# hahnyuan/PTQ4ViT

Hardware: AMD Instinct MI355X
Metric: calibration throughput (wrapped modules calibrated per second), ViT-B/224 W8A8, 32 calibration images (higher is better)
Workload: dtype int8

## Files before the change

ptq4vit_amd/csrc/p4v_api.hip:

```cpp
#include <hip/hip_runtime.h>

#include <algorithm>
#include <atomic>
#include <climits>
#include <cstdarg>
#include <cstdio>
#include <condition_variable>
#include <cstring>
#include <deque>
#include <functional>
#include <thread>
#include <mutex>
#include <string>
#include <unordered_map>
#include <type_traits>
#include <vector>

#include "../../include/ptq4vit_hip.h"
#include "../../include/ptq4vit_hip_debug.h"
#include "p4v_kernels.h"

using namespace p4v;

namespace {
// ... 75 lines not shown

struct StatRec { hipEvent_t a, b; int kind; double macs, alg; int stage, gx, gz; double ms, bytes; };
thread_local double g_alg_bytes = 0;
thread_local double g_alg_macs_cand = 0;
thread_local double g_exec_frac = 1.0;
thread_local bool g_stat_on = false;
thread_local std::vector<StatRec> g_stat_recs;
thread_local std::vector<StatRec> g_stat_done;
thread_local bool g_b1_keep = false;
thread_local std::vector<float> g_b1_totals;
enum PruneStage { STAGE_FULL = 0, STAGE_A = 1, STAGE_B1 = 2, STAGE_B2 = 3, STAGE_A2 = 4 };
thread_local int g_stage = STAGE_FULL;
thread_local p4v_kernel_stats g_stats = {};
thread_local long g_memo_hits = 0, g_memo_misses = 0;
std::atomic<long long> g_prune_cnt[4];
constexpr int VARIANT_KEPT = 1 | 2 | 4 | 2048 | 32768 | 65536 | 131072 | 524288 | 1048576 | 2097152 | 4194304 | 8388608 | 134217728;
std::atomic<int> g_variant_word{0};
#define g_variant (g_variant_word.load(std::memory_order_relaxed) & 0x3fffffff)
#define g_force_v1 ((g_variant_word.load(std::memory_order_relaxed) >> 30) & 1)
std::atomic<int> g_tune[16];
enum { TUNE_CG6 = 0, TUNE_CG2 = 1, TUNE_CG2G = 2, TUNE_CG7 = 3, TUNE_PRINT = 4, TUNE_ORDER7 = 5, TUNE_P6 = 6, TUNE_PLANE_GIB = 7, TUNE_EPI6W = 8,
       TUNE_LOOSE_PCT = 9, TUNE_SLICE_DIV = 10, TUNE_SLICE_SMALL = 11, TUNE_B1_PATH = 12, TUNE_TIER2 = 13, TUNE_TIER2_DIV = 14, TUNE_LOOSE_ROWS = 15 };
inline bool tune_b1_removed(int v) { return v == 1 || v == 2 || v == 3 || v == 5 || v == 6 || v == 8 || v == 10 || v == 12; }
inline int tune(int k) { return g_tune[k].load(std::memory_order_relaxed); }
inline bool b1_previous() { return tune(TUNE_B1_PATH) == 4; }

inline int ws_aligned(const void* p) {
    return ((uintptr_t)p % WS_ALIGN) == 0 ? 0 : fail(P4V_ERR_INVALID, "d_workspace must be aligned to %zu bytes", WS_ALIGN);
}

struct Group;
// ... 421 lines not shown
    if (total >= (1L << 31)) return fail(P4V_ERR_UNSUPPORTED, "operand plane too large for k_pack (%ld 16-element runs)", total);
    const int groups = cdiv((p.crange && live_max > 0) ? std::min(p.C, live_max) : p.C, PACK_CG);
    const long cap = !p.crange ? 256L * 64 : live_max > 0 ? std::max(256L * 12, 256L * 64 / groups) : 256L * 12;
    const int blocks = (int)std::min<long>(cdiv(total, 256), cap);
    if (p.mode == PACK_TWIN_I8) {
        if (sizeof(T) != 1 || p.C != 1 || p.c_inner != 0 || !p.scales || p.conv || p.zdiv > 0)
            return fail(P4V_ERR_UNSUPPORTED, "merged twin plane: one fixed row-major int8 plane only");
        return enqueue(c, KERN(PackParams, k_pack_twin), dim3(blocks), dim3(256), 0, p);
    }
    const bool single = sizeof(T) == 1 && pack1_ok(p, live_max) && !g_pack_general.load(std::memory_order_relaxed);
    if (tune(TUNE_PRINT) > 1) fprintf(stderr, "[p4v] %s stage %d: Z %d Rp %d Kp %d C %d crange %d done %d live_max %d layout %d grid %d x %d\n", single ? "k_pack1" : "k_pack", g_stage, p.Z, p.Rp, p.Kp, p.C, p.crange != nullptr, p.done != nullptr, live_max, p.c_inner, blocks, single ? 1 : groups);
    if (single) return enqueue(c, KERN(PackParams, k_pack1), dim3(blocks), dim3(256), 0, p);
    return enqueue(c, KERN_T(PackParams, k_pack, T), dim3(blocks, groups), dim3(256), 0, p);
}

inline int lockstep(const Ctx& c, int kind) {
    if (!c.grp) return 1;
    const int seen = (kind >= 0 && kind < 16) ? c.grp->last_par[kind] : 0;
    return std::max(1, seen > 0 ? seen : c.par);
}
inline int cu_slots(const Ctx& c, int slots, int kind) { return std::max(8, slots / lockstep(c, kind)); }
#define P4V_EPI4(epi, X)                                   \
    switch (epi) {                                         \
        case EPI_SQ_W: { constexpr int E = EPI_SQ_W; X; }  \
        case EPI_SQ: { constexpr int E = EPI_SQ; X; }      \
        case EPI_ABS: { constexpr int E = EPI_ABS; X; }    \
        default: { constexpr int E = EPI_W_SQ; X; }        \
    }

template <typename T, bool TWIN> int launch_sweep_epi(Ctx& c, const SweepParams& p, int epi, int cgroups, const StatInfo* si) {
// ... 47 lines not shown
    HIPCHK(hipStreamSynchronize(c.st));
    std::vector<unsigned long long> h(n);
    HIPCHK(hipMemcpy(h.data(), g_trace, n * 8, hipMemcpyDeviceToHost));
    FILE* f = fopen(getenv("P4V_TRACE_FILE"), "ab");
    unsigned long long hdr[4] = {0xABCDull, grid.x, grid.z, (unsigned long long)ktiles};
    fwrite(hdr, 8, 4, f); fwrite(h.data(), 8, n, f); fclose(f);
    return 0;
}
#endif

inline StatInfo stat_info(int kind, double macs, double alg, int gx, int gz, double bytes) {
    return StatInfo{kind, macs * g_exec_frac, alg * g_exec_frac, g_stage, gx, gz, bytes};
}

enum SweepKind { SK_BOUND, SK_SWEEP6, SK_SWEEP5, SK_SWEEP7, SK_SWEEP7_TWIN, SK_SWEEP7_MERGED, SK_SWEEP9, SK_SWEEP8, SK_SWEEP2G, SK_SWEEP2,
                 SK_GENERIC_I8, SK_GENERIC_F32, SK_COUNT };
constexpr int SWEEP_RECORD_KIND[SK_COUNT] = {12, 2, 5, 3, 4, 4, 6, 7, 8, 9, 0, 1};
inline bool sweep_stationary(SweepKind k) { return k == SK_SWEEP6 || k == SK_SWEEP5; }
inline bool sweep_large_k(SweepKind k) { return k == SK_SWEEP7 || k == SK_SWEEP7_TWIN || k == SK_SWEEP7_MERGED; }

int launch_sweep5(Ctx& c, const Sweep3Params& p, int epi, int cgroups) {
    if (c.dry) return 0;
    const int per = 2 * cdiv(p.c1 - p.c0, 2 * cgroups);
    const size_t lds = (size_t)p.ktiles * SW2_TILE + (size_t)SW5_NP * 2 * SW2_TILE + (size_t)per * 8 * sizeof(float) * 2 + 256;
    dim3 grid(p.stiles * p.ttiles, 1, cgroups), block(512);
#ifdef P4V_TRACE
    CHK(trace_attach(const_cast<Sweep3Params&>(p)));
#endif
    const StatInfo si = stat_info(SWEEP_RECORD_KIND[SK_SWEEP5], (double)p.stiles * 128 * (double)p.ttiles * 128 * (double)p.ldk * (p.c1 - p.c0), g_alg_macs_cand * (p.c1 - p.c0),
                                  (int)grid.x, (int)grid.z, g_alg_bytes);
    const StatInfo* sp = &si;
    P4V_EPI4(epi, CHK(enqueue(c, KERN_T(Sweep3Params, k_sweep5, E), grid, block, lds, p, sp)); break)
// ... 97 lines not shown
    const int per_max = (int)((160 * 1024 - SW7_NS * SW7_STAGE - 256) / 192);
    cgroups = std::max(cgroups, cdiv(nc, per_max));
    const int per = cdiv(nc, cgroups);
    const size_t lds = (size_t)SW7_NS * SW7_STAGE + (size_t)per * 192 + 256;
    Sweep7Params q = p;
    q.cgroups = cgroups;
    dim3 grid(p.rtiles * p.ctiles * cgroups, 1, 1);
    const StatInfo si = stat_info(SWEEP_RECORD_KIND[twin ? SK_SWEEP7_TWIN : SK_SWEEP7], (double)p.rtiles * 256 * (double)p.ctiles * 256 * (double)p.ldk * nc, g_alg_macs_cand * nc,
                                  (int)grid.x, (int)grid.z, g_alg_bytes);
    const StatInfo* sp = &si;
    return twin == 2 ? launch_sweep7_epi<2>(c, q, epi, grid, lds, sp) : twin ? launch_sweep7_epi<1>(c, q, epi, grid, lds, sp) : launch_sweep7_epi<0>(c, q, epi, grid, lds, sp);
}

int launch_sweep(Ctx& c, const SweepParams& p, SweepKind kind, bool twin, int epi, int cgroups) {
    if (c.dry) return 0;
    const double kelems = (double)p.ldk / (kind == SK_GENERIC_F32 ? 4 : 1);
    const int tiles = p.mtiles * p.ntiles;
    auto record = [&](int gx) {
        return stat_info(SWEEP_RECORD_KIND[kind], (double)p.mtiles * SW_BM * (double)p.ntiles * SW_BN * kelems * p.Z * (p.c1 - p.c0) * (twin ? 2 : 1),
                         g_alg_macs_cand * (p.c1 - p.c0), gx, cgroups, g_alg_bytes);
    };
    switch (kind) {
        case SK_BOUND: {
            const bool prev = b1_previous();
            const StatInfo si = record(tiles * (prev ? 2 : 1));
            const dim3 grid(tiles * (prev ? 2 : 1)), block(256);
            if (prev) P4V_EPI4(epi, return enqueue(c, KERN_T(SweepParams, k_bound, E, 1), grid, block, 0, p, &si))
            P4V_EPI4(epi, return enqueue(c, KERN_T(SweepParams, k_bound, E, 2), grid, block, 0, p, &si))
        }
        case SK_SWEEP9: {
            const StatInfo si = record(p.halves);
// ... 6 lines not shown
        case SK_SWEEP2G: {
            const StatInfo si = record(tiles);
            return twin ? launch_sweep2g_epi<true>(c, p, epi, cgroups, &si) : launch_sweep2g_epi<false>(c, p, epi, cgroups, &si);
        }
        case SK_SWEEP2: {
            const StatInfo si = record(tiles);
            return twin ? launch_sweep2_epi<true>(c, p, epi, cgroups, &si) : launch_sweep2_epi<false>(c, p, epi, cgroups, &si);
        }
        case SK_GENERIC_I8: {
            const StatInfo si = record(tiles);
            return twin ? launch_sweep_epi<int8_t, true>(c, p, epi, cgroups, &si) : launch_sweep_epi<int8_t, false>(c, p, epi, cgroups, &si);
        }
        case SK_GENERIC_F32: {
            const StatInfo si = record(tiles);
            return twin ? launch_sweep_epi<float, true>(c, p, epi, cgroups, &si) : launch_sweep_epi<float, false>(c, p, epi, cgroups, &si);
        }
        default: return fail(P4V_ERR_INVALID, "launch_sweep: family %d has a launcher of its own", (int)kind);
    }
}

int launch_finish(Ctx& c, const FinishParams& p) {
    return enqueue(c, KERN(FinishParams, k_finish), dim3(p.C, p.nj), dim3(256), 0, p);
}

int launch_finish_cos(Ctx& c, const FinishCosParams& p) {
    const int gy = p.j_mode == 3 ? cdiv(p.S, 256) : p.nj;
    return enqueue(c, KERN(FinishCosParams, k_finish_cos), dim3(p.C, gy), dim3(p.j_mode == 3 ? 256 : 1024), 0, p);
}

int launch_select(Ctx& c, const SelectParams& p_) {
// ... 224 lines not shown
    CHK(launch_pass_select(c, ps, scores));
    c.ws.off = mark;
    return 0;
}

struct SweepPlan {
    SweepKind kind;
    bool pairs;
    bool merged7;
    bool b64;
    bool fast_cos;
    bool epi6_on;
    const int* rblk;
    const int* rblk_z;
    int esz, Kp, Mp, Np, NpB;
    long row_plane1, col_plane1, exp_plane;
    int chunk, chunk_al; size_t slack;
    int cin_exp, cin_fix;
    size_t zero_bias_n, epi7_n;
    int s6_stiles, s6_ttiles; size_t epi6_bytes;
    bool a_search;
    long part_cs;
    long p_zs, p_cs; int NpP;
    int s3_groups, cos6_Sp;
    int h9;
    long fin_zs; int fin_ld, fin_rows, fin_cols, fin_jdiv;
};

int sweep9_halves(const Pass& ps, int ktiles) {
    const int epi = ps.epi;
    if (ktiles != 1 || ps.twin || ps.row.expanded == ps.col.expanded || epi == EPI_STORE || epi == EPI_FWD || epi == EPI_COS) return 0;
// ... 5 lines not shown
    if (halves > 32 / SW9_NW) return 0;
    const double waste = (double)rup(ps.Mrows, 128) * rup(ps.Ncols, 128) / ((double)rup(ps.Mrows, 16) * rup(ps.Ncols, 16));
    return (waste >= 1.4 || (g_variant & 1048576)) ? halves : 0;
}
bool sweep8_ok(const Pass& ps, int ktiles) {
    return ktiles == 1 && !ps.twin && ps.row.expanded != ps.col.expanded && ps.epi != EPI_STORE && ps.epi != EPI_FWD && ps.epi != EPI_COS &&
           !(g_variant & 65536);
}
bool sweep2g_ok(const Pass& ps, int ktiles) {
    return ps.col.expanded && !ps.row.expanded && ktiles >= 16 && ps.o_bs == 0 && ps.o_nbs == 0 && ps.epi != EPI_COS;
}

int plan_sweep(const Ctx& c, const Pass& ps, SweepPlan& pl) {
    pl = SweepPlan{};
    const int esz = pl.esz = ps.i8 ? 1 : 4;
    const int Kp = pl.Kp = (int)rup(ps.K, 64 / esz);
    const int ktiles = Kp * esz / SW_BKB;
    const long K64 = rup(ps.K, 64);
    const bool cosm = ps.epi == EPI_COS, i8v2 = ps.i8 && !g_force_v1;
    const bool one_expanded = ps.row.expanded != ps.col.expanded, plain_out = ps.o_bs == 0 && ps.o_nbs == 0;
    const bool scale32 = ps.sb_mode != 1 || ps.s_cs == 1 || ps.sb_div % 32 == 0;
    const bool score32 = ps.j_mode == 0 || (ps.j_mode == 1 && (ps.nj == 1 || ps.j_div % 32 == 0));
    const bool blocks64 = (ps.s_cs == 1 || ps.sb_div % 64 == 0) && (ps.j_mode == 0 || (ps.j_mode == 1 && (ps.nj == 1 || ps.j_div % 64 == 0)));
    const bool bound = ps.bound_kernel && i8v2 && !ps.twin && ps.Z == 1 && !ps.stores() && !cosm && plain_out && ps.bias_axis == 0 &&
                       (ps.sb_mode == 0 || ps.sb_mode == 1) && score32 && scale32 && (ps.eq_n == 1 || ps.crange);
    const bool stat_ok = !bound && !ps.stores() && i8v2 && !ps.twin && (!cosm || ps.cos6) && !(g_variant & 4) && ps.Z == 1 &&
                         ps.sb_mode == 1 && blocks64 && one_expanded && K64 <= 768 && plain_out;
    const bool regs6 = stat_ok && sweep6_supported(ktiles);
    if (ps.cos6 && !regs6) return fail(P4V_ERR_UNSUPPORTED, "cosine pass planned for k_sweep6 does not qualify for it");
    const bool big7 = !bound && !stat_ok && !ps.stores() && i8v2 && (!cosm || ps.cos7) && !(g_variant & 32768) && ps.Z == 1 &&
                      K64 >= 1024 && K64 % 256 == 0 && (long)ps.Mrows * ps.o_ms * 4 < (1L << 32) && ps.sb_mode == 1 && scale32 && score32 &&
                      one_expanded && !(ps.twin && (ps.row.expanded || ps.row2.expanded)) &&
                      plain_out && ps.o_ns == 1 && ps.Ncols % 32 == 0 && ps.o_ms % 4 == 0 &&
                      (c.dry || ((((unsigned long long)ps.O) | ((unsigned long long)(ps.G ? ps.G : ps.O))) & 15) == 0) && ps.bias_axis == 0;
    if (ps.cos7 && (!big7 || ps.twin)) return fail(P4V_ERR_UNSUPPORTED, "cosine pass planned for k_sweep7 does not qualify for it");
    const bool fast = !stat_ok && i8v2 && !cosm && scale32 && (score32 || ps.j_mode == 2);
    pl.fast_cos = cosm && !stat_ok && !big7 && i8v2 && !ps.stores() && tune(TUNE_B1_PATH) != 7 && scale32;
    pl.pairs = stat_ok && !regs6;
    pl.merged7 = big7 && ps.twin && ps.twin_disjoint && !(g_variant & 2097152);
    pl.kind = bound ? SK_BOUND : regs6 ? SK_SWEEP6 : stat_ok ? SK_SWEEP5 :
              big7 ? (pl.merged7 ? SK_SWEEP7_MERGED : ps.twin ? SK_SWEEP7_TWIN : SK_SWEEP7) :
              !(fast || pl.fast_cos) ? (ps.i8 ? SK_GENERIC_I8 : SK_GENERIC_F32) :
              (fast && sweep8_ok(ps, ktiles)) ? SK_SWEEP8 : (fast && sweep2g_ok(ps, ktiles)) ? SK_SWEEP2G : SK_SWEEP2;
    const bool blk_ranges = ps.crange && ps.crange_blk && tune(TUNE_B1_PATH) != 9;
    pl.rblk = (blk_ranges && regs6 && !ps.row.expanded && ps.j_mode == 1 && ps.nj == ps.s_cs && ps.j_div == ps.sb_div) ? ps.crange_blk : nullptr;
    pl.rblk_z = (blk_ranges && !stat_ok && ps.j_mode == 2 && ps.nj == ps.j_div && ps.Z > 1 && !cosm && !ps.stores() && !bound && K64 < 1024)
                    ? ps.crange_blk : nullptr;
    const int Mp = pl.Mp = (int)rup(ps.Mrows, big7 ? (ps.twin ? 128 : 256) : (regs6 && !ps.row.expanded) ? 256 : SW_BM);
    const int Np = pl.Np = (int)rup(ps.Ncols, big7 ? 256 : (regs6 && !ps.col.expanded) ? 256 : SW_BM);
    pl.b64 = fast && !big7 && !bound && ps.Z > 1 && !ps.col_zs_shared && ps.Ncols <= 64 && ktiles >= 2 && ktiles <= 15 && !ps.stores();
    pl.NpB = pl.b64 ? 64 : Np;
    pl.row_plane1 = (long)(ps.row_zs_shared ? 1 : ps.Z) * Mp * Kp * esz;
    pl.col_plane1 = (long)(ps.col_zs_shared ? 1 : ps.Z) * pl.NpB * Kp * esz;
    pl.exp_plane = ps.row.expanded ? pl.row_plane1 : pl.col_plane1;
    pl.chunk = (int)std::max<long>(1, std::min<long>(ps.eq_n, PLANE_BUDGET / std::max<long>(1, pl.exp_plane)));
    if (pl.pairs && pl.chunk > 1) pl.chunk &= ~1;
    pl.chunk_al = pl.pairs ? ((pl.chunk + 1) & ~1) : pl.chunk;
    pl.slack = stat_ok ? 4096 : 0;
    pl.cin_exp = bound ? 3 : stat_ok ? (pl.pairs ? 2 : 1) : 0;
    pl.cin_fix = (bound || regs6) ? 3 : 0;
    pl.zero_bias_n = stat_ok ? (size_t)std::max(Mp, Np) : 0;
    pl.epi7_n = big7 ? (size_t)Mp * Np * 2 : 0;
    const bool a_search = pl.a_search = ps.row.expanded;
    pl.s6_stiles = (a_search ? Np : Mp) / 256; pl.s6_ttiles = (int)cdiv(a_search ? ps.Mrows : ps.Ncols, 64);
    pl.epi6_on = regs6 && (a_search || ps.cos6 || tune(TUNE_EPI6W) == 1);
    pl.epi6_bytes = pl.epi6_on ? (size_t)pl.s6_stiles * pl.s6_ttiles * (256 * 64 * 8) : 0;
    const int MT = Mp / 64, s3_slabs = (a_search ? Np : Mp) / 64, s3_groups = pl.s3_groups = (a_search ? Mp : Np) / 32;
    const int NpP = pl.NpP = stat_ok ? s3_groups : fast ? Np / 32 : Np;
    const int MT7 = big7 ? (Mp / (ps.twin ? 128 : 256)) * 4 : 0;
    const bool cosp = ps.cos6 || ps.cos7;
// ... 18 lines not shown
        if (cosp) pl.fin_zs = (long)FS * cos6_Sp * 3;
        pl.fin_ld = cosp ? cos6_Sp : Np; pl.fin_rows = cosp ? FS : MT; pl.fin_cols = cosp ? ps.Mrows : ps.Ncols;
        pl.fin_jdiv = std::max(1, ps.cos_j_div);
    }
    return 0;
}
inline SweepKind chunk_kind(const SweepPlan& pl, int nc) { return (pl.kind == SK_SWEEP2G && nc < 2) ? SK_SWEEP2 : pl.kind; }

struct PassBufs {
    char* row; char* row2; char* col;
    float* part; float* S1; float* S2; float* scores; float* zero_bias; float* epi7; float* epi6;
    PlaneCache* pc; EpiCache* ec;
};
int pass_workspace(Ctx& c, const Pass& ps, const SweepPlan& pl, PassBufs& b) {
    PlaneCache* pc = b.pc = (ps.cache && pl.chunk >= ps.eq_n && !ps.stores() && ps.row.expanded != ps.col.expanded &&
                             !(ps.twin && ps.row2.expanded) && pl.exp_plane * (long)ps.eq_n <= PLANE_CACHE_MAX) ? ps.cache : nullptr;
    if (pc && !pc->assigned) {
        pc->buf = c.ws.get_top((size_t)pl.exp_plane * pl.chunk_al + pl.slack);
        pc->done = reinterpret_cast<unsigned char*>(c.ws.get_top((size_t)rup(ps.eq_n, 256)));
        pc->assigned = true; pc->valid = false;
        if (!c.dry && pc->done) CHK(q_fill(c, pc->done, 0, (size_t)ps.eq_n));
    }
    b.row = ps.row.prepacked ? (char*)ps.row.plane :
            (pc && ps.row.expanded) ? pc->buf : c.ws.get<char>((size_t)pl.row_plane1 * (ps.row.expanded ? pl.chunk_al : 1) + pl.slack);
    b.row2 = !ps.twin ? nullptr : ps.row2.prepacked ? (char*)ps.row2.plane : c.ws.get<char>((size_t)pl.row_plane1 * (ps.row2.expanded ? pl.chunk : 1));
    b.col = ps.col.prepacked ? (char*)ps.col.plane :
            (pc && ps.col.expanded) ? pc->buf : c.ws.get<char>((size_t)pl.col_plane1 * (ps.col.expanded ? pl.chunk_al : 1) + pl.slack);
    b.part = c.ws.get<float>((size_t)pl.part_cs * ps.eq_n);
    b.S1 = !ps.use_s1 ? nullptr : ps.S1_pre ? ps.S1_pre : c.ws.get<float>((size_t)ps.eq_n * ps.s_cs);
    b.S2 = !(ps.use_s1 && ps.twin) ? nullptr : ps.S2_pre ? ps.S2_pre : c.ws.get<float>((size_t)ps.eq_n * ps.s_cs);
    b.scores = ps.scores_keep ? ps.scores_keep : c.ws.get<float>((size_t)ps.eq_n * std::max(1, ps.nj));
    b.zero_bias = (pl.zero_bias_n && !ps.bias) ? c.ws.get<float>(pl.zero_bias_n) : nullptr;
    b.epi7 = pl.epi7_n ? c.ws.get<float>(pl.epi7_n) : nullptr;
    EpiCache* ec = b.ec = (pl.epi6_on && ps.ecache && (long)pl.epi6_bytes <= PLANE_CACHE_MAX) ? ps.ecache : nullptr;
    if (ec && !ec->assigned) {
        ec->buf = c.ws.get_top(pl.epi6_bytes);
        ec->assigned = true; ec->valid = false;
    }
    b.epi6 = !pl.epi6_on ? nullptr : ec ? reinterpret_cast<float*>(ec->buf) : c.ws.get<float>(pl.epi6_bytes / 4);
    if (!c.ws.ok()) return fail(P4V_ERR_WORKSPACE, "workspace too small: need >= %zu bytes", c.ws.off);
    return 0;
}

int pack_operand(Ctx& c, const Pass& ps, const SweepPlan& pl, const PassBufs& b, const Operand& op, char* buf, bool col, int c0, int nc) {
    PackParams pk = op.pk;
    pk.Rp = col ? pl.NpB : pl.Mp; pk.Kp = pl.Kp; pk.dst = buf;
    pk.Z = (col ? ps.col_zs_shared : ps.row_zs_shared) ? 1 : ps.Z;
    pk.C = op.expanded ? nc : 1;
    pk.c_inner = op.expanded ? pl.cin_exp : pl.cin_fix;
    if (op.expanded && pk.scales) pk.scales += (long)c0 * pk.sc_cs;
    if (op.expanded && ps.crange) {
        pk.crange = ps.crange; pk.c_base = c0;
        pk.done = (b.pc && b.pc->done) ? b.pc->done : nullptr;
    }
    int live_max = -1;
    if (pk.crange && ps.host_hi > ps.host_lo) live_max = std::max(0, std::min(ps.host_hi, c0 + nc) - std::max(ps.host_lo, c0));
    else if (pk.crange && ps.host_len > 0) live_max = std::min(ps.host_len, nc);
    return ps.i8 ? launch_pack<int8_t>(c, pk, live_max) : launch_pack<float>(c, pk, live_max);
}
int pack_expanded(Ctx& c, const Pass& ps, const SweepPlan& pl, const PassBufs& b, int c0, int nc) {
    PlaneCache* pc = b.pc;
    const bool packed = pc && pc->valid;
    if (ps.row.expanded && !packed) CHK(pack_operand(c, ps, pl, b, ps.row, b.row, false, c0, nc));
    if (ps.twin && ps.row2.expanded) CHK(pack_operand(c, ps, pl, b, ps.row2, b.row2, false, c0, nc));
    if (ps.col.expanded && !packed) CHK(pack_operand(c, ps, pl, b, ps.col, b.col, true, c0, nc));
    if (pc && !ps.crange && !packed) {
        pc->valid = true;
        if (!c.dry && pc->done) CHK(q_fill(c, pc->done, 1, (size_t)ps.eq_n));
    }
    return 0;
}

// ... 143 lines not shown
    q.ldk = pl.Kp; q.ktiles = pl.Kp / SW_BKB;
    q.S1 = b.S1; q.S2 = b.S2; q.s_cs = ps.s_cs; q.sb_div = ps.s_cs > 1 ? std::max(1, ps.sb_div) : (1 << 30);
    q.E = b.epi7;
    q.c0 = c0; q.c1 = c0 + nc; q.crange = ps.crange;
    q.part = b.part; q.p_cs = pl.p_cs; q.NG = ps.cos7 ? pl.cos6_Sp : pl.NpP;
    q.rtiles = pl.Np / 256; q.ctiles = pl.Mp / (ps.twin ? 128 : 256);
    int cg7 = choose_cgroups((long)q.rtiles * q.ctiles, nc, q.ktiles + 3, cu_slots(c, 256, SWEEP_RECORD_KIND[ps.twin ? SK_SWEEP7_TWIN : SK_SWEEP7]), 6.0, 0.62, 100);
    if (tune(TUNE_CG7) > 0) cg7 = std::max(1, std::min(nc, tune(TUNE_CG7)));
    q.order = tune(TUNE_ORDER7) > 0 ? tune(TUNE_ORDER7) - 1 : 1;
    if (tune(TUNE_PRINT) > 0) fprintf(stderr, "[p4v] sweep7 tiles %d x %d ktiles %d cand %d twin %d -> cgroups %d\n", q.rtiles, q.ctiles, q.ktiles, nc, (int)ps.twin, cg7);
    if (pl.kind == SK_SWEEP7_MERGED) { q.twin_s = ps.row.pk.scales; q.C2 = b.row2; }
    return launch_sweep7(c, q, pl.kind == SK_SWEEP7_MERGED ? 2 : ps.twin ? 1 : 0, ps.epi, cg7);
}

int sweep_chunk_tiled(Ctx& c, const Pass& ps, const SweepPlan& pl, const PassBufs& b, SweepKind kind, int c0, int nc) {
    const int esz = pl.esz, Mp = pl.Mp, Np = pl.Np, Kp = pl.Kp;
    SweepParams sp{};
    sp.a_cs = ps.row.expanded ? pl.row_plane1 : 0;
    sp.A = b.row - (long)c0 * sp.a_cs;
    sp.a_zs = ps.row_zs_shared ? 0 : (long)Mp * Kp * esz;
    if (ps.twin) {
        sp.a2_cs = ps.row2.expanded ? pl.row_plane1 : 0;
        sp.A2 = b.row2 - (long)c0 * sp.a2_cs;
        sp.a2_zs = sp.a_zs;
    }
    sp.b_cs = ps.col.expanded ? pl.col_plane1 : 0;
    sp.B = b.col - (long)c0 * sp.b_cs;
    sp.b_zs = ps.col_zs_shared ? 0 : (long)pl.NpB * Kp * esz;
    sp.b_rows = pl.b64 ? 64 : 0;
    sp.ldk = Kp * esz; sp.ktiles = sp.ldk / SW_BKB;
    sp.S1 = b.S1; sp.S2 = b.S2; sp.s_cs = ps.s_cs; sp.sb_mode = ps.sb_mode; sp.sb_div = std::max(1, ps.sb_div);
    sp.bias = ps.bias; sp.bias_axis = ps.bias_axis; sp.bias_zs = ps.bias_zs;
    sp.O = ps.O; sp.Wt = ps.G ? ps.G : ps.O; sp.wt_mode = ps.wt_mode;
    sp.o_zs = ps.o_zs; sp.o_bs = ps.o_bs; sp.o_ms = ps.o_ms; sp.o_nbs = ps.o_nbs; sp.o_ns = ps.o_ns;
    sp.o_inner = ps.o_inner > 0 ? ps.o_inner : INT_MAX;
    sp.o_ninner = ps.o_ninner > 0 ? ps.o_ninner : INT_MAX;
    sp.M = ps.Mrows; sp.N = ps.Ncols; sp.Z = ps.Z; sp.c0 = c0; sp.c1 = c0 + nc; sp.crange = ps.crange;
    sp.crange_blk = pl.rblk_z; sp.cb_div = std::max(1, ps.j_div);
    sp.part = b.part; sp.p_cs = pl.p_cs; sp.p_zs = pl.p_zs; sp.Np = pl.NpP;
    sp.mtiles = Mp / SW_BM; sp.ntiles = Np / SW_BN;
    sp.dbg = g_variant & 3;
    sp.store = ps.store_out;
    const long wgs = (long)sp.mtiles * sp.ntiles * ps.Z;
    int cgroups;
    switch (kind) {
        case SK_GENERIC_I8: case SK_GENERIC_F32:
            cgroups = choose_cgroups(wgs, nc, sp.ktiles, cu_slots(c, 512, SWEEP_RECORD_KIND[kind]), 20.0, ps.i8 ? 1.6 : 2.6);
            break;
        case SK_SWEEP9:
            sp.halves = pl.h9;
            sp.rows_p_stream = sp.a_cs == 0 ? Np : Mp;
            cgroups = choose_cgroups((long)pl.h9 * ps.Z, nc, 1, cu_slots(c, SW9_NW == 4 ? 512 : 256, SWEEP_RECORD_KIND[SK_SWEEP9]), 12.0, 0.9);
            break;
        case SK_BOUND:
            sp.bound = 1;
            sp.dbg = tune(TUNE_B1_PATH) >= 16 ? (tune(TUNE_B1_PATH) >> 4) : 0;
            sp.A = b.row; sp.B = b.col; sp.a_cs = sp.b_cs = 0;
            [[fallthrough]];
        default:
            cgroups = choose_cgroups(wgs, nc, sp.ktiles, cu_slots(c, ps.twin ? 256 : 512, SWEEP_RECORD_KIND[SK_SWEEP2]), ps.twin ? 40.0 : 25.0, ps.twin ? 0.45 : 0.40);
    }
    const bool tuned = kind != SK_GENERIC_I8 && kind != SK_GENERIC_F32 && !pl.fast_cos && !ps.stores();
    if (tuned) {
        const char* g = kind == SK_SWEEP2G ? "g" : "";
        if (const int t_ = tune(kind == SK_SWEEP2G ? TUNE_CG2G : TUNE_CG2); t_ > 0) cgroups = std::max(1, std::min(nc, t_));
        if (tune(TUNE_PRINT) > 0) fprintf(stderr, "[p4v] sweep2%s tiles %d x %d z %d ktiles %d cand %d twin %d -> cgroups %d\n", g, sp.mtiles, sp.ntiles, ps.Z, sp.ktiles, nc, (int)ps.twin, cgroups);
    }
    return launch_sweep(c, sp, kind, ps.twin, ps.epi, cgroups);
}

int finish_pass(Ctx& c, const Pass& ps, const SweepPlan& pl, const PassBufs& b) {
    if (ps.epi == EPI_COS) {
        FinishCosParams fp{b.part, pl.p_cs, pl.fin_zs, pl.fin_ld, pl.fin_rows, ps.cos_ZB, ps.cos_ZV, pl.fin_cols, ps.eq_n,
                           ps.cos_j_mode, pl.fin_jdiv, ps.nj, ps.norm, b.scores};
        return launch_finish_cos(c, fp);
    }
    FinishParams fp{b.part, pl.p_cs, pl.fin_zs, pl.fin_ld, pl.fin_rows, ps.Z, pl.fin_cols, ps.eq_n, ps.j_mode, pl.fin_jdiv, ps.nj, ps.norm,
// ... 2756 lines not shown
```

ptq4vit_amd/csrc/p4v_kernels.h:

```cpp
#pragma once
#include <hip/hip_runtime.h>
#include <stdint.h>
#include <type_traits>

namespace p4v {

typedef int v4i __attribute__((ext_vector_type(4)));
typedef int v16i __attribute__((ext_vector_type(16)));
typedef float v4f __attribute__((ext_vector_type(4)));
typedef float v16f __attribute__((ext_vector_type(16)));
typedef float v2f __attribute__((ext_vector_type(2)));

#ifndef P4V_GROUP_KERNARG
#define P4V_GROUP_KERNARG (4096 - 256)
#endif
template <typename P> struct GroupArgs {
    static constexpr int CAP_RAW = (P4V_GROUP_KERNARG - 16) / (int)(sizeof(P) + 16);
    static constexpr int CAP = CAP_RAW > 64 ? 64 : CAP_RAW;
    int n;
    unsigned off[CAP + 1];
    unsigned gx[CAP], gy[CAP], gz[CAP];
    P p[CAP];
};
#define P4V_BIDX uint3{blockIdx.x, blockIdx.y, blockIdx.z}
// ... 933 lines not shown
                nn += __shfl_xor(nn, 32);
                oo += __shfl_xor(oo, 32);
                if (g == 0) {
                    float* q = cos_part(p, c, z, mt * 2 + wr, n0 + wc * 32 + l31);
                    q[0] = dot; q[1] = nn; q[2] = oo;
                }
            }
            zero_acc();
        }
    }
}
template <typename T, bool TWIN, int EPI>
__global__ __launch_bounds__(512, 2) void k_sweep(SweepParams p) { k_sweep_body<T, TWIN, EPI>(p, P4V_BIDX, P4V_GDIM); }
template <typename T, bool TWIN, int EPI>
__global__ __launch_bounds__(512, 2) void k_sweep_g(GroupArgs<SweepParams> a) { P4V_GROUP_ENTER(a); k_sweep_body<T, TWIN, EPI>(a.p[m_], vb_, vg_); }

static constexpr int SW2_NS = 4;
static constexpr int SW2_TILE = 128 * 64;

__device__ __forceinline__ void glds16(const void* g, void* l) {
    __builtin_amdgcn_global_load_lds((const __attribute__((address_space(1))) void*)g,
                                     (__attribute__((address_space(3))) void*)l, 16, 0, 0);
}
template <int OFF> __device__ __forceinline__ void glds16_imm(const void* g, void* l) {
    __builtin_amdgcn_global_load_lds((const __attribute__((address_space(1))) void*)g,
                                     (__attribute__((address_space(3))) void*)l, 16, OFF, 0);
}

__device__ __forceinline__ float wave_sum_dpp(float v) {
    auto dpp = [](float x, auto ctrl, auto rmask) __attribute__((always_inline)) {
// ... 3604 lines not shown
```

Before: 689.9.

## Add bf16x3-split MFMA sweep path for fp32 passes with quantized expanded operand

Adds a new sweep kind for non-int8 passes whose expanded column operand is symmetrically quantized to at most 256 levels. That operand is packed as exact bf16 integers, and the raw fp32 row operand is split into three bf16 parts. A new kernel runs bf16 MFMA for the hi and lo parts and applies the candidate scale in the epilogue, replacing the generic fp32 sweep. The aim is to move fp32 GEMM work onto bf16 matrix cores, at the cost of three MFMAs per tile and larger row-plane storage. Precision depends on the three-way split. Workspace sizing is adjusted to fit the new plane sizes.

```diff
diff --git a/ptq4vit_amd/csrc/p4v_api.hip b/ptq4vit_amd/csrc/p4v_api.hip
--- a/ptq4vit_amd/csrc/p4v_api.hip
+++ b/ptq4vit_amd/csrc/p4v_api.hip
@@ -113,7 +113,7 @@
 thread_local p4v_kernel_stats g_stats = {};
 thread_local long g_memo_hits = 0, g_memo_misses = 0;
 std::atomic<long long> g_prune_cnt[4];
-constexpr int VARIANT_KEPT = 1 | 2 | 4 | 2048 | 32768 | 65536 | 131072 | 524288 | 1048576 | 2097152 | 4194304 | 8388608 | 134217728;
+constexpr int VARIANT_KEPT = 1 | 2 | 4 | 16 | 2048 | 32768 | 65536 | 131072 | 524288 | 1048576 | 2097152 | 4194304 | 8388608 | 134217728;
 std::atomic<int> g_variant_word{0};
 #define g_variant (g_variant_word.load(std::memory_order_relaxed) & 0x3fffffff)
 #define g_force_v1 ((g_variant_word.load(std::memory_order_relaxed) >> 30) & 1)
@@ -565,6 +565,17 @@
     return enqueue(c, KERN_T(PackParams, k_pack, T), dim3(blocks, groups), dim3(256), 0, p);
 }
 
+int launch_pack_bf3(Ctx& c, const PackParams& p, bool expanded, int live_max) {
+    if (c.dry) return 0;
+    if (p.crange && live_max == 0) return 0;
+    const long total = (long)p.Z * p.Rp * (p.Kp / 16);
+    if (total >= (1L << 31)) return fail(P4V_ERR_UNSUPPORTED, "operand plane too large for k_pack_bf3 (%ld 16-element runs)", total);
+    if (!expanded) return enqueue(c, KERN(PackParams, k_pack_bf3x), dim3((unsigned)std::min<long>(cdiv(total, 256), 256L * 64)), dim3(256), 0, p);
+    const int groups = cdiv((p.crange && live_max > 0) ? std::min(p.C, live_max) : p.C, PACK_CG);
+    const long cap = !p.crange ? 256L * 64 : live_max > 0 ? std::max(256L * 12, 256L * 64 / groups) : 256L * 12;
+    return enqueue(c, KERN(PackParams, k_pack_bf3q), dim3((unsigned)std::min<long>(cdiv(total, 256), cap), groups), dim3(256), 0, p);
+}
+
 inline int lockstep(const Ctx& c, int kind) {
     if (!c.grp) return 1;
     const int seen = (kind >= 0 && kind < 16) ? c.grp->last_par[kind] : 0;
@@ -642,8 +653,8 @@
 }
 
 enum SweepKind { SK_BOUND, SK_SWEEP6, SK_SWEEP5, SK_SWEEP7, SK_SWEEP7_TWIN, SK_SWEEP7_MERGED, SK_SWEEP9, SK_SWEEP8, SK_SWEEP2G, SK_SWEEP2,
-                 SK_GENERIC_I8, SK_GENERIC_F32, SK_COUNT };
-constexpr int SWEEP_RECORD_KIND[SK_COUNT] = {12, 2, 5, 3, 4, 4, 6, 7, 8, 9, 0, 1};
+                 SK_GENERIC_I8, SK_GENERIC_F32, SK_BF3, SK_COUNT };
+constexpr int SWEEP_RECORD_KIND[SK_COUNT] = {12, 2, 5, 3, 4, 4, 6, 7, 8, 9, 0, 1, 1};
 inline bool sweep_stationary(SweepKind k) { return k == SK_SWEEP6 || k == SK_SWEEP5; }
 inline bool sweep_large_k(SweepKind k) { return k == SK_SWEEP7 || k == SK_SWEEP7_TWIN || k == SK_SWEEP7_MERGED; }
 
@@ -771,7 +782,7 @@
 
 int launch_sweep(Ctx& c, const SweepParams& p, SweepKind kind, bool twin, int epi, int cgroups) {
     if (c.dry) return 0;
-    const double kelems = (double)p.ldk / (kind == SK_GENERIC_F32 ? 4 : 1);
+    const double kelems = kind == SK_BF3 ? 3.0 * p.ldk / 2 : (double)p.ldk / (kind == SK_GENERIC_F32 ? 4 : 1);
     const int tiles = p.mtiles * p.ntiles;
     auto record = [&](int gx) {
         return stat_info(SWEEP_RECORD_KIND[kind], (double)p.mtiles * SW_BM * (double)p.ntiles * SW_BN * kelems * p.Z * (p.c1 - p.c0) * (twin ? 2 : 1),
@@ -808,6 +819,11 @@
         case SK_GENERIC_F32: {
             const StatInfo si = record(tiles);
             return twin ? launch_sweep_epi<float, true>(c, p, epi, cgroups, &si) : launch_sweep_epi<float, false>(c, p, epi, cgroups, &si);
+        }
+        case SK_BF3: {
+            const StatInfo si = record(tiles);
+            const dim3 grid(tiles, p.Z, cgroups), block(512);
+            P4V_EPI4(epi, return enqueue(c, KERN_T(SweepParams, k_sweep_bf3, E), grid, block, 2 * BF3_STAGE, p, &si))
         }
         default: return fail(P4V_ERR_INVALID, "launch_sweep: family %d has a launcher of its own", (int)kind);
     }
@@ -1062,7 +1078,9 @@
     const int* rblk;
     const int* rblk_z;
     int esz, Kp, Mp, Np, NpB;
+    int esz_row, esz_col;
     long row_plane1, col_plane1, exp_plane;
+    long row_alloc1, col_alloc1, exp_alloc;
     int chunk, chunk_al; size_t slack;
     int cin_exp, cin_fix;
     size_t zero_bias_n, epi7_n;
@@ -1098,8 +1116,16 @@
 int plan_sweep(const Ctx& c, const Pass& ps, SweepPlan& pl) {
     pl = SweepPlan{};
     const int esz = pl.esz = ps.i8 ? 1 : 4;
-    const int Kp = pl.Kp = (int)rup(ps.K, 64 / esz);
-    const int ktiles = Kp * esz / SW_BKB;
+    const PackParams& cpk = ps.col.pk;
+    const bool bf3_ok = !ps.i8 && !ps.twin && !ps.stores() && ps.epi != EPI_COS && !ps.use_s1 &&
+                     !ps.row.expanded && !ps.row.prepacked && ps.row.pk.mode == PACK_RAW &&
+                     ps.col.expanded && cpk.mode == PACK_SYM && cpk.hi - cpk.lo <= 255 && cpk.lo >= -128 && cpk.hi <= 128 &&
+                     (cpk.blk_mode == 0 || (cpk.blk_mode == 1 && !cpk.blk_div2 && cpk.blk_div >= 1 && cpk.sc_cs == cpk.nblk_r)) &&
+                     ps.sb_mode == 0 && ps.s_cs == 1;
+    const bool bf3 = bf3_ok && !(g_variant & 16);
+    pl.esz_row = bf3 ? 6 : esz; pl.esz_col = bf3 ? 2 : esz;
+    const int Kp = pl.Kp = (int)rup(ps.K, bf3 ? BF3_BK : 64 / esz);
+    const int ktiles = bf3 ? Kp / BF3_BK : Kp * esz / SW_BKB;
     const long K64 = rup(ps.K, 64);
     const bool cosm = ps.epi == EPI_COS, i8v2 = ps.i8 && !g_force_v1;
     const bool one_expanded = ps.row.expanded != ps.col.expanded, plain_out = ps.o_bs == 0 && ps.o_nbs == 0;
@@ -1124,7 +1150,7 @@
     pl.merged7 = big7 && ps.twin && ps.twin_disjoint && !(g_variant & 2097152);
     pl.kind = bound ? SK_BOUND : regs6 ? SK_SWEEP6 : stat_ok ? SK_SWEEP5 :
               big7 ? (pl.merged7 ? SK_SWEEP7_MERGED : ps.twin ? SK_SWEEP7_TWIN : SK_SWEEP7) :
-              !(fast || pl.fast_cos) ? (ps.i8 ? SK_GENERIC_I8 : SK_GENERIC_F32) :
+              !(fast || pl.fast_cos) ? (ps.i8 ? SK_GENERIC_I8 : bf3 ? SK_BF3 : SK_GENERIC_F32) :
               (fast && sweep8_ok(ps, ktiles)) ? SK_SWEEP8 : (fast && sweep2g_ok(ps, ktiles)) ? SK_SWEEP2G : SK_SWEEP2;
     const bool blk_ranges = ps.crange && ps.crange_blk && tune(TUNE_B1_PATH) != 9;
     pl.rblk = (blk_ranges && regs6 && !ps.row.expanded && ps.j_mode == 1 && ps.nj == ps.s_cs && ps.j_div == ps.sb_div) ? ps.crange_blk : nullptr;
@@ -1134,10 +1160,17 @@
     const int Np = pl.Np = (int)rup(ps.Ncols, big7 ? 256 : (regs6 && !ps.col.expanded) ? 256 : SW_BM);
     pl.b64 = fast && !big7 && !bound && ps.Z > 1 && !ps.col_zs_shared && ps.Ncols <= 64 && ktiles >= 2 && ktiles <= 15 && !ps.stores();
     pl.NpB = pl.b64 ? 64 : Np;
-    pl.row_plane1 = (long)(ps.row_zs_shared ? 1 : ps.Z) * Mp * Kp * esz;
-    pl.col_plane1 = (long)(ps.col_zs_shared ? 1 : ps.Z) * pl.NpB * Kp * esz;
+    pl.row_plane1 = (long)(ps.row_zs_shared ? 1 : ps.Z) * Mp * Kp * pl.esz_row;
+    pl.col_plane1 = (long)(ps.col_zs_shared ? 1 : ps.Z) * pl.NpB * Kp * pl.esz_col;
     pl.exp_plane = ps.row.expanded ? pl.row_plane1 : pl.col_plane1;
-    pl.chunk = (int)std::max<long>(1, std::min<long>(ps.eq_n, PLANE_BUDGET / std::max<long>(1, pl.exp_plane)));
+    pl.row_alloc1 = pl.row_plane1; pl.col_alloc1 = pl.col_plane1;
+    if (bf3_ok) {
+        const long Kf = rup(ps.K, 16), Kb = rup(ps.K, BF3_BK);
+        pl.row_alloc1 = (long)(ps.row_zs_shared ? 1 : ps.Z) * Mp * std::max(Kf * 4, Kb * 6);
+        pl.col_alloc1 = (long)(ps.col_zs_shared ? 1 : ps.Z) * pl.NpB * std::max(Kf * 4, Kb * 2);
+    }
+    pl.exp_alloc = ps.row.expanded ? pl.row_alloc1 : pl.col_alloc1;
+    pl.chunk = (int)std::max<long>(1, std::min<long>(ps.eq_n, PLANE_BUDGET / std::max<long>(1, pl.exp_alloc)));
     if (pl.pairs && pl.chunk > 1) pl.chunk &= ~1;
     pl.chunk_al = pl.pairs ? ((pl.chunk + 1) & ~1) : pl.chunk;
     pl.slack = stat_ok ? 4096 : 0;
@@ -1186,18 +1219,18 @@
 };
 int pass_workspace(Ctx& c, const Pass& ps, const SweepPlan& pl, PassBufs& b) {
     PlaneCache* pc = b.pc = (ps.cache && pl.chunk >= ps.eq_n && !ps.stores() && ps.row.expanded != ps.col.expanded &&
-                             !(ps.twin && ps.row2.expanded) && pl.exp_plane * (long)ps.eq_n <= PLANE_CACHE_MAX) ? ps.cache : nullptr;
+                             !(ps.twin && ps.row2.expanded) && pl.exp_alloc * (long)ps.eq_n <= PLANE_CACHE_MAX) ? ps.cache : nullptr;
     if (pc && !pc->assigned) {
-        pc->buf = c.ws.get_top((size_t)pl.exp_plane * pl.chunk_al + pl.slack);
+        pc->buf = c.ws.get_top((size_t)pl.exp_alloc * pl.chunk_al + pl.slack);
         pc->done = reinterpret_cast<unsigned char*>(c.ws.get_top((size_t)rup(ps.eq_n, 256)));
         pc->assigned = true; pc->valid = false;
         if (!c.dry && pc->done) CHK(q_fill(c, pc->done, 0, (size_t)ps.eq_n));
     }
     b.row = ps.row.prepacked ? (char*)ps.row.plane :
-            (pc && ps.row.expanded) ? pc->buf : c.ws.get<char>((size_t)pl.row_plane1 * (ps.row.expanded ? pl.chunk_al : 1) + pl.slack);
+            (pc && ps.row.expanded) ? pc->buf : c.ws.get<char>((size_t)pl.row_alloc1 * (ps.row.expanded ? pl.chunk_al : 1) + pl.slack);
     b.row2 = !ps.twin ? nullptr : ps.row2.prepacked ? (char*)ps.row2.plane : c.ws.get<char>((size_t)pl.row_plane1 * (ps.row2.expanded ? pl.chunk : 1));
     b.col = ps.col.prepacked ? (char*)ps.col.plane :
-            (pc && ps.col.expanded) ? pc->buf : c.ws.get<char>((size_t)pl.col_plane1 * (ps.col.expanded ? pl.chunk_al : 1) + pl.slack);
+            (pc && ps.col.expanded) ? pc->buf : c.ws.get<char>((size_t)pl.col_alloc1 * (ps.col.expanded ? pl.chunk_al : 1) + pl.slack);
     b.part = c.ws.get<float>((size_t)pl.part_cs * ps.eq_n);
     b.S1 = !ps.use_s1 ? nullptr : ps.S1_pre ? ps.S1_pre : c.ws.get<float>((size_t)ps.eq_n * ps.s_cs);
     b.S2 = !(ps.use_s1 && ps.twin) ? nullptr : ps.S2_pre ? ps.S2_pre : c.ws.get<float>((size_t)ps.eq_n * ps.s_cs);
@@ -1228,6 +1261,7 @@
     int live_max = -1;
     if (pk.crange && ps.host_hi > ps.host_lo) live_max = std::max(0, std::min(ps.host_hi, c0 + nc) - std::max(ps.host_lo, c0));
     else if (pk.crange && ps.host_len > 0) live_max = std::min(ps.host_len, nc);
+    if (pl.kind == SK_BF3) return launch_pack_bf3(c, pk, op.expanded, live_max);
     return ps.i8 ? launch_pack<int8_t>(c, pk, live_max) : launch_pack<float>(c, pk, live_max);
 }
 int pack_expanded(Ctx& c, const Pass& ps, const SweepPlan& pl, const PassBufs& b, int c0, int nc) {
@@ -1401,11 +1435,11 @@
 }
 
 int sweep_chunk_tiled(Ctx& c, const Pass& ps, const SweepPlan& pl, const PassBufs& b, SweepKind kind, int c0, int nc) {
-    const int esz = pl.esz, Mp = pl.Mp, Np = pl.Np, Kp = pl.Kp;
+    const int Mp = pl.Mp, Np = pl.Np, Kp = pl.Kp;
     SweepParams sp{};
     sp.a_cs = ps.row.expanded ? pl.row_plane1 : 0;
     sp.A = b.row - (long)c0 * sp.a_cs;
-    sp.a_zs = ps.row_zs_shared ? 0 : (long)Mp * Kp * esz;
+    sp.a_zs = ps.row_zs_shared ? 0 : (long)Mp * Kp * pl.esz_row;
     if (ps.twin) {
         sp.a2_cs = ps.row2.expanded ? pl.row_plane1 : 0;
         sp.A2 = b.row2 - (long)c0 * sp.a2_cs;
@@ -1413,10 +1447,15 @@
     }
     sp.b_cs = ps.col.expanded ? pl.col_plane1 : 0;
     sp.B = b.col - (long)c0 * sp.b_cs;
-    sp.b_zs = ps.col_zs_shared ? 0 : (long)pl.NpB * Kp * esz;
+    sp.b_zs = ps.col_zs_shared ? 0 : (long)pl.NpB * Kp * pl.esz_col;
     sp.b_rows = pl.b64 ? 64 : 0;
-    sp.ldk = Kp * esz; sp.ktiles = sp.ldk / SW_BKB;
+    sp.ldk = Kp * pl.esz_col; sp.ktiles = kind == SK_BF3 ? Kp / BF3_BK : sp.ldk / SW_BKB;
     sp.S1 = b.S1; sp.S2 = b.S2; sp.s_cs = ps.s_cs; sp.sb_mode = ps.sb_mode; sp.sb_div = std::max(1, ps.sb_div);
+    if (kind == SK_BF3) {
+        const PackParams& cpk = ps.col.pk;
+        if (!c.dry && !cpk.scales) return fail(P4V_ERR_INVALID, "k_sweep_bf3: the expanded operand has no candidate table");
+        sp.S1 = cpk.scales; sp.s_cs = cpk.sc_cs; sp.sb_mode = cpk.blk_mode == 1 ? 1 : 0; sp.sb_div = std::max(1, cpk.blk_div);
+    }
     sp.bias = ps.bias; sp.bias_axis = ps.bias_axis; sp.bias_zs = ps.bias_zs;
     sp.O = ps.O; sp.Wt = ps.G ? ps.G : ps.O; sp.wt_mode = ps.wt_mode;
     sp.o_zs = ps.o_zs; sp.o_bs = ps.o_bs; sp.o_ms = ps.o_ms; sp.o_nbs = ps.o_nbs; sp.o_ns = ps.o_ns;
@@ -1434,6 +1473,9 @@
         case SK_GENERIC_I8: case SK_GENERIC_F32:
             cgroups = choose_cgroups(wgs, nc, sp.ktiles, cu_slots(c, 512, SWEEP_RECORD_KIND[kind]), 20.0, ps.i8 ? 1.6 : 2.6);
             break;
+        case SK_BF3:
+            cgroups = choose_cgroups(wgs, nc, sp.ktiles, cu_slots(c, 256, SWEEP_RECORD_KIND[kind]), 20.0, 1.2);
+            break;
         case SK_SWEEP9:
             sp.halves = pl.h9;
             sp.rows_p_stream = sp.a_cs == 0 ? Np : Mp;
@@ -1447,7 +1489,7 @@
         default:
             cgroups = choose_cgroups(wgs, nc, sp.ktiles, cu_slots(c, ps.twin ? 256 : 512, SWEEP_RECORD_KIND[SK_SWEEP2]), ps.twin ? 40.0 : 25.0, ps.twin ? 0.45 : 0.40);
     }
-    const bool tuned = kind != SK_GENERIC_I8 && kind != SK_GENERIC_F32 && !pl.fast_cos && !ps.stores();
+    const bool tuned = kind != SK_GENERIC_I8 && kind != SK_GENERIC_F32 && kind != SK_BF3 && !pl.fast_cos && !ps.stores();
     if (tuned) {
         const char* g = kind == SK_SWEEP2G ? "g" : "";
         if (const int t_ = tune(kind == SK_SWEEP2G ? TUNE_CG2G : TUNE_CG2); t_ > 0) cgroups = std::max(1, std::min(nc, t_));
diff --git a/ptq4vit_amd/csrc/p4v_kernels.h b/ptq4vit_amd/csrc/p4v_kernels.h
--- a/ptq4vit_amd/csrc/p4v_kernels.h
+++ b/ptq4vit_amd/csrc/p4v_kernels.h
@@ -971,6 +971,217 @@
 __global__ __launch_bounds__(512, 2) void k_sweep(SweepParams p) { k_sweep_body<T, TWIN, EPI>(p, P4V_BIDX, P4V_GDIM); }
 template <typename T, bool TWIN, int EPI>
 __global__ __launch_bounds__(512, 2) void k_sweep_g(GroupArgs<SweepParams> a) { P4V_GROUP_ENTER(a); k_sweep_body<T, TWIN, EPI>(a.p[m_], vb_, vg_); }
+
+static constexpr int BF3_BK = 64;
+static constexpr int BF3_AROW = 3 * BF3_BK * 2 + 16, BF3_BROW = BF3_BK * 2 + 16;
+static constexpr int BF3_STAGE = SW_BM * BF3_AROW + SW_BN * BF3_BROW;
+typedef __bf16 v8bf __attribute__((ext_vector_type(8)));
+
+__device__ __forceinline__ void bf3_split(float x, unsigned (&h)[3]) {
+    if (!(fabsf(x) <= 3.4028234664e38f)) {
+        h[0] = (x != x) ? 0x7fc0u : (__builtin_bit_cast(unsigned, x) >> 16); h[1] = 0u; h[2] = 0u;
+        return;
+    }
+    float r = x;
+#pragma unroll
+    for (int i = 0; i < 3; ++i) {
+        const unsigned u = __builtin_bit_cast(unsigned, r) & 0xffff0000u;
+        h[i] = u >> 16;
+        r -= __builtin_bit_cast(float, u);
+    }
+}
+
+__device__ __forceinline__ void k_pack_bf3x_body(const PackParams& p, const uint3 blockIdx, const uint3 gridDim) {
+    const unsigned kchunks = p.Kp / 16;
+    const unsigned total = (unsigned)p.Z * p.Rp * kchunks;
+    for (unsigned i = blockIdx.x * 256u + threadIdx.x; i < total; i += gridDim.x * 256u) {
+        const unsigned row = i / kchunks;
+        const int kc = (int)(i - row * kchunks);
+        const int z = (int)(row / (unsigned)p.Rp);
+        const int r = (int)(row - (unsigned)z * p.Rp);
+        const float* zbase = p.zdiv > 0 ? p.src + (long)(z / p.zdiv) * p.s_z2 + (long)(z % p.zdiv) * p.s_z : p.src + (long)z * p.s_z;
+        float x[16];
+        pack_load16(p, zbase, r, kc, x);
+        unsigned w[3][8];
+#pragma unroll
+        for (int e = 0; e < 16; e += 2) {
+            unsigned a[3], b[3];
+            bf3_split(x[e], a); bf3_split(x[e + 1], b);
+#pragma unroll
+            for (int j = 0; j < 3; ++j) w[j][e >> 1] = a[j] | (b[j] << 16);
+        }
+        char* d = reinterpret_cast<char*>(p.dst) + (long)row * p.Kp * 6 + (long)(kc >> 2) * (3 * BF3_BK * 2) + (kc & 3) * 32;
+#pragma unroll
+        for (int j = 0; j < 3; ++j) {
+            *reinterpret_cast<v4i*>(d + j * BF3_BK * 2) = v4i{(int)w[j][0], (int)w[j][1], (int)w[j][2], (int)w[j][3]};
+            *reinterpret_cast<v4i*>(d + j * BF3_BK * 2 + 16) = v4i{(int)w[j][4], (int)w[j][5], (int)w[j][6], (int)w[j][7]};
+        }
+    }
+}
+__global__ __launch_bounds__(256) void k_pack_bf3x(PackParams p) { k_pack_bf3x_body(p, P4V_BIDX, P4V_GDIM); }
+__global__ __launch_bounds__(256) void k_pack_bf3x_g(GroupArgs<PackParams> a) { P4V_GROUP_ENTER(a); k_pack_bf3x_body(a.p[m_], vb_, vg_); }
+
+__device__ __forceinline__ void k_pack_bf3q_body(const PackParams& p, const uint3 blockIdx, const uint3 gridDim) {
+    const unsigned kchunks = p.Kp / 16;
+    const unsigned total = (unsigned)p.Z * p.Rp * kchunks;
+    int cbeg = blockIdx.y * PACK_CG, cend = min(p.C, cbeg + PACK_CG);
+    if (p.crange) {
+        const int a = max(p.crange[0] - p.c_base, 0), b = min(p.crange[1] - p.c_base, p.C);
+        cbeg = a + (int)blockIdx.y * PACK_CG; cend = min(b, cbeg + PACK_CG);
+        if (cbeg >= cend) return;
+    }
+    unsigned need = (1u << (cend - cbeg)) - 1u;
+    if (p.crange && p.done) {
+        for (int j = 0; j < PACK_CG; ++j)
+            if (cbeg + j < cend && p.done[cbeg + j]) need &= ~(1u << j);
+        if (!need) return;
+    }
+    const float flo = (float)p.lo, fhi = (float)p.hi;
+    for (unsigned i = blockIdx.x * 256u + threadIdx.x; i < total; i += gridDim.x * 256u) {
+        const unsigned row = i / kchunks;
+        const int kc = (int)(i - row * kchunks);
+        const int z = (int)(row / (unsigned)p.Rp);
+        const int r = (int)(row - (unsigned)z * p.Rp);
+        const float* zbase = p.zdiv > 0 ? p.src + (long)(z / p.zdiv) * p.s_z2 + (long)(z % p.zdiv) * p.s_z : p.src + (long)z * p.s_z;
+        float x[16];
+        pack_load16(p, zbase, r, kc, x);
+        const int blk0 = pack_blk(p, z, r, 0);
+        for (int j = 0; j < PACK_CG; ++j) {
+            const int c = cbeg + j;
+            if (c >= cend) break;
+            if (!((need >> j) & 1u)) continue;
+            const float s = p.scales[c * p.sc_cs + blk0];
+            unsigned w[8];
+#pragma unroll
+            for (int e = 0; e < 16; ++e) {
+                const float q = rintf(x[e] / s);
+                const float v = (r < p.R && kc * 16 + e < p.K) ? (q != q ? q : fminf(fmaxf(q, flo), fhi)) : 0.0f;
+                const unsigned hb = (v != v) ? 0x7fc0u : (__builtin_bit_cast(unsigned, v) >> 16);
+                w[e >> 1] = (e & 1) ? (w[e >> 1] | (hb << 16)) : hb;
+            }
+            char* d = reinterpret_cast<char*>(p.dst) + ((((long)c * p.Z + z) * p.Rp + r) * p.Kp + (long)kc * 16) * 2;
+            __builtin_nontemporal_store(v4i{(int)w[0], (int)w[1], (int)w[2], (int)w[3]}, reinterpret_cast<v4i*>(d));
+            __builtin_nontemporal_store(v4i{(int)w[4], (int)w[5], (int)w[6], (int)w[7]}, reinterpret_cast<v4i*>(d + 16));
+        }
+    }
+}
+__global__ __launch_bounds__(256) void k_pack_bf3q(PackParams p) { k_pack_bf3q_body(p, P4V_BIDX, P4V_GDIM); }
+__global__ __launch_bounds__(256) void k_pack_bf3q_g(GroupArgs<PackParams> a) { P4V_GROUP_ENTER(a); k_pack_bf3q_body(a.p[m_], vb_, vg_); }
+
+template <int EPI>
+__device__ __forceinline__ void k_sweep_bf3_body(const SweepParams& p, const uint3 blockIdx, const uint3 gridDim) {
+    extern __shared__ __attribute__((aligned(16))) char smem[];
+    const int tid = threadIdx.x, lane = tid & 63, wid = tid >> 6;
+    const int wr = wid >> 2, wc = wid & 3;
+    const int g = lane >> 5, l31 = lane & 31;
+
+    const int nwg = p.mtiles * p.ntiles;
+    const int t = xcd_remap(blockIdx.x, nwg);
+    const int mt = t % p.mtiles, nt = t / p.mtiles;
+    const int z = blockIdx.y;
+    const int m0 = mt * SW_BM, n0 = nt * SW_BN;
+    const CandSpan cspan = cand_span(p.c0, p.c1, p.crange, blockIdx.z, gridDim.z, p.crange_blk, [&] { return z % p.cb_div; });
+    const int c_lo = cspan.lo, c_hi = cspan.hi;
+    if (c_lo >= c_hi) return;
+
+    float u[2][16], w[2][16];
+    const int n = n0 + wc * 32 + l31;
+    const bool ncol_ok = n < p.N;
+    const float* biasz = p.bias ? p.bias + (long)z * p.bias_zs : nullptr;
+    const float bias_n = (biasz && ncol_ok && p.bias_axis == 0) ? biasz[n] : 0.0f;
+    const int nc = min(n, p.N - 1);
+    const long ncol_off = (long)z * p.o_zs + (long)(nc / p.o_ninner) * p.o_nbs + (long)(nc % p.o_ninner) * p.o_ns;
+    tile_targets<EPI>(p, [&](int mc) { return ncol_off + (long)(mc / p.o_inner) * p.o_bs + (long)(mc % p.o_inner) * p.o_ms; },
+                      m0 + wr * 64, g, ncol_ok, bias_n, biasz, p.bias_axis, u, w);
+    const int sb = scale_block(p, n, z);
+
+    const long lda = 3L * p.ldk;
+    const char* gA = (const char*)p.A + (long)z * p.a_zs + (long)m0 * lda;
+    const char* gB = (const char*)p.B + (long)z * p.b_zs + (long)n0 * p.ldk;
+    int a_go[6], a_lo[6], b_go[2], b_lo[2];
+#pragma unroll
+    for (int j = 0; j < 6; ++j) { const int pc = tid + j * 512, row = pc / 24, cc = pc % 24; a_go[j] = row * (int)lda + cc * 16; a_lo[j] = row * BF3_AROW + cc * 16; }
+#pragma unroll
+    for (int j = 0; j < 2; ++j) { const int pc = tid + j * 512, row = pc >> 3, cc = pc & 7; b_go[j] = row * p.ldk + cc * 16; b_lo[j] = SW_BM * BF3_AROW + row * BF3_BROW + cc * 16; }
+
+    const int total = (c_hi - c_lo) * p.ktiles;
+    v4i ra[6], rb[2];
+    auto gload = [&](int it) {
+        const int c = c_lo + it / p.ktiles, kt = it % p.ktiles;
+        const char* a = gA + (long)c * p.a_cs + (long)kt * (3 * BF3_BK * 2);
+        const char* b = gB + (long)c * p.b_cs + (long)kt * (BF3_BK * 2);
+#pragma unroll
+        for (int j = 0; j < 6; ++j) ra[j] = *reinterpret_cast<const v4i*>(a + a_go[j]);
+#pragma unroll
+        for (int j = 0; j < 2; ++j) rb[j] = *reinterpret_cast<const v4i*>(b + b_go[j]);
+    };
+    auto lstore = [&](int stage) {
+        char* s = smem + stage * BF3_STAGE;
+#pragma unroll
+        for (int j = 0; j < 6; ++j) *reinterpret_cast<v4i*>(s + a_lo[j]) = ra[j];
+#pragma unroll
+        for (int j = 0; j < 2; ++j) *reinterpret_cast<v4i*>(s + b_lo[j]) = rb[j];
+    };
+
+    v16f hi[2], lo[2];
+    auto zero_acc = [&]() {
+#pragma unroll
+        for (int i = 0; i < 2; ++i)
+#pragma unroll
+            for (int r = 0; r < 16; ++r) { hi[i][r] = 0.0f; lo[i][r] = 0.0f; }
+    };
+    zero_acc();
+
+    const int fa = (wr * 64 + l31) * BF3_AROW + g * 16;
+    const int fb = SW_BM * BF3_AROW + (wc * 32 + l31) * BF3_BROW + g * 16;
+
+    gload(0);
+    lstore(0);
+    __syncthreads();
+
+    for (int it = 0; it < total; ++it) {
+        const int stage = it & 1;
+        if (it + 1 < total) gload(it + 1);
+        const char* s = smem + stage * BF3_STAGE;
+#pragma unroll
+        for (int h = 0; h < BF3_BK / 16; ++h) {
+            const v8bf b = *reinterpret_cast<const v8bf*>(s + fb + h * 32);
+#pragma unroll
+            for (int i = 0; i < 2; ++i) {
+                const char* ap = s + fa + i * 32 * BF3_AROW + h * 32;
+                const v8bf a1 = *reinterpret_cast<const v8bf*>(ap);
+                const v8bf a2 = *reinterpret_cast<const v8bf*>(ap + BF3_BK * 2);
+                const v8bf a3 = *reinterpret_cast<const v8bf*>(ap + 2 * BF3_BK * 2);
+                hi[i] = __builtin_amdgcn_mfma_f32_32x32x16_bf16(a1, b, hi[i], 0, 0, 0);
+                lo[i] = __builtin_amdgcn_mfma_f32_32x32x16_bf16(a2, b, lo[i], 0, 0, 0);
+                lo[i] = __builtin_amdgcn_mfma_f32_32x32x16_bf16(a3, b, lo[i], 0, 0, 0);
+            }
+        }
+        if (it + 1 < total) lstore(stage ^ 1);
+        __syncthreads();
+
+        if ((it + 1) % p.ktiles == 0) {
+            const int c = c_lo + it / p.ktiles;
+            const float s1 = p.S1[c * p.s_cs + sb];
+            float colsum = 0.0f;
+#pragma unroll
+            for (int i = 0; i < 2; ++i)
+#pragma unroll
+                for (int r = 0; r < 16; ++r) {
+                    const float d = u[i][r] - (hi[i][r] + lo[i][r]) * s1;
+                    metric_add<EPI>(colsum, w[i][r], d);
+                }
+            colsum += __shfl_xor(colsum, 32);
+            if (g == 0)
+                p.part[(long)c * p.p_cs + (long)z * p.p_zs + (long)(mt * 2 + wr) * p.Np + n0 + wc * 32 + l31] = colsum;
+            zero_acc();
+        }
+    }
+}
+template <int EPI>
+__global__ __launch_bounds__(512, 1) void k_sweep_bf3(SweepParams p) { k_sweep_bf3_body<EPI>(p, P4V_BIDX, P4V_GDIM); }
+template <int EPI>
+__global__ __launch_bounds__(512, 1) void k_sweep_bf3_g(GroupArgs<SweepParams> a) { P4V_GROUP_ENTER(a); k_sweep_bf3_body<EPI>(a.p[m_], vb_, vg_); }
 
 static constexpr int SW2_NS = 4;
 static constexpr int SW2_TILE = 128 * 64;
```

Result: no change. 690.7 (median of 2 runs) (+0.1%).
